# microsoft/Sora

Measured on AMD Instinct MI355X. Metric: IQ Msamples/s through 802.11a 54 Mbps RX PHY, higher is better.
Workload: dtype int16 IQ / u8 path metrics

## Files before the change

sora_amd/csrc/dev_vit16.h:

```cpp
#pragma once
#include <hip/hip_runtime.h>
#include "kernels.h"
#include "dev_viterbi.h"

namespace sora {
namespace {

template <int WIN, int LOOK> struct Geom16 {
    static constexpr int kMaxWalk = (WIN + LOOK + 7) / 8 + 2;
    static constexpr int P = kMaxWalk;
    static constexpr int kPathBytes = 40;
};

template <int WIN, int LOOK> struct Lds16 {
    uint16_t ring[Geom16<WIN, LOOK>::P][4][64];
    union {
        uint32_t udump[4][64];
        uint16_t ops[4][24][2];
        uint16_t ops2[2][4][24][2];
    };
    uint32_t path[8][Geom16<WIN, LOOK>::kPathBytes / 4];
};

constexpr unsigned kW[4] = { 0u, 21u, 42u, 63u };

__device__ __forceinline__ unsigned v_of_lane(unsigned l)
{
    const unsigned b0 = l & 1u, b1 = (l >> 1) & 1u, b2 = (l >> 2) & 1u, b3 = (l >> 3) & 1u;
    const unsigned c3 = b2, c1 = b3, c0 = b0 ^ c3, c2 = b1 ^ c3;
    return c0 | (c1 << 1) | (c2 << 2) | (c3 << 3);
}
__device__ __forceinline__ unsigned lane_of_v(unsigned v)
{
    const unsigned c0 = v & 1u, c1 = (v >> 1) & 1u, c2 = (v >> 2) & 1u, c3 = (v >> 3) & 1u;
    return c0 ^ (c2 << 1) ^ (c1 << 3) ^ (c3 ? 7u : 0u);
}
__device__ __forceinline__ unsigned rev6u(unsigned x) { return __brev(x) >> 26; }

template <int CTRL> __device__ __forceinline__ unsigned dppx(unsigned v) { return (unsigned)__builtin_amdgcn_update_dpp(0, (int)v, CTRL, 0xF, 0xF, true); }

__device__ __forceinline__ unsigned partner(unsigned v, int ph)
{
    switch (ph) {
    case 0: return dppx<0x140>(v);
    case 1: return dppx<0x1B>(v);
    case 2: return dppx<0x141>(v);
    case 3: return dppx<0x4E>(v);
    case 4: return dppx<0x128>(v);
    default: return dppx<0xB1>(v);
    }
}

struct Vit16 {
    unsigned U[4];
    unsigned MX[24];
    unsigned MY[6];
    unsigned sadr[3][4];
};

template <int WHICH, int P>
__device__ __forceinline__ void acs16(Vit16& V, int t24, unsigned a, unsigned b, unsigned pos512[3])
{
    const int ph = t24 % 6, k = t24 % 8;
    const unsigned Kp = (WHICH == 0 ? 14u : 7u) * kFld + (kOne << k);
    unsigned bm;
    if (WHICH == 0)      bm = (a ^ V.MX[t24]) + (b ^ V.MY[ph]);
    else if (WHICH == 1) bm = a ^ V.MX[t24];
    else                 bm = b ^ V.MX[t24];
    const unsigned bo = Kp - bm;
    const int rx = ph == 0 ? 2 : ph == 1 ? 1 : 0;
    unsigned N[4];
#pragma unroll
    for (int i = 0; i < 4; i++) {
        const unsigned X = V.U[i], Y = partner(V.U[i ^ rx], ph);
        const bool wb = (kW[i] >> (5 - ph)) & 1u;
        N[i] = wb ? pk_min16(X + bo, Y + bm) : pk_min16(X + bm, Y + bo);
    }
#pragma unroll
    for (int i = 0; i < 4; i++) V.U[i] = N[i];
    if (k == 7) {
        const int jb = t24 / 8;
#pragma unroll
        for (int i = 0; i < 4; i++) {
            const unsigned w = bank_word(V.U[i]);
            const unsigned addr = V.sadr[jb][i] + pos512[jb];
            asm volatile("ds_write_b16 %0, %1" : : "v"(addr), "v"(w) : "memory");
            V.U[i] &= 0xFE00FE00u;
        }
    }
}

__device__ __forceinline__ unsigned row_min_u32(unsigned v)
{
    v = min(v, dppx<0xB1>(v)); v = min(v, dppx<0x4E>(v)); v = min(v, dppx<0x141>(v)); v = min(v, dppx<0x128>(v));
    return v;
}
__device__ __forceinline__ unsigned row_pkmin(unsigned v)
{
    v = pk_min16(v, dppx<0xB1>(v)); v = pk_min16(v, dppx<0x4E>(v)); v = pk_min16(v, dppx<0x141>(v)); v = pk_min16(v, dppx<0x128>(v));
    return v;
}
__device__ __forceinline__ unsigned wave_min_u32(unsigned v) { return (unsigned)__builtin_amdgcn_readfirstlane((int)dpp_min_u32_wave(v)); }
__device__ __forceinline__ unsigned wave_max_u32(unsigned v) { return ~wave_min_u32(~v); }

template <int CR, int WIN, int LOOK, int BITS>
struct Forward16 {
    static constexpr int P = Geom16<WIN, LOOK>::P, GB = Puncture<CR>::GB, GS = Puncture<CR>::GS, CW = Puncture<CR>::CW;
    static constexpr int NV = Puncture<CR>::NV;
    struct Chunk { uint32_t v[CW]; };
    struct Raw { SoftRaw r[NV]; };

    Vit16 V;
    unsigned row, half;
    uint32_t my_j;
    SoftCursor<BITS, CW> cur[NV];
    uint32_t my_base;
    const uint8_t* soft;
    uint16_t* my_ops;
    const uint4* row_ops;
    uint32_t pos;
    unsigned pos512[3];
    uint32_t tr, nsteps;
    uint32_t next_thr;
    bool all_done;

    __device__ __forceinline__ void init(Lds16<WIN, LOOK>& S, const uint8_t* __restrict__ soft_, uint32_t my_soft_off, uint32_t my_first, uint32_t my_last, unsigned start,
                                         uint32_t nsteps_)
    {
        const unsigned lane = threadIdx.x & 63, l16 = lane & 15;
        row = lane >> 4; half = lane & 1u;
        const unsigned v0 = v_of_lane(l16);
        nsteps = nsteps_;
#pragma unroll
        for (int i = 0; i < 4; i++) V.U[i] = (v0 ^ kW[i]) == 0 ? 0u : start;
        const unsigned ring_base = (unsigned)(uintptr_t)&S.ring[0][0][0];
#pragma unroll
        for (int jb = 0; jb < 3; jb++)
#pragma unroll
            for (int i = 0; i < 4; i++) V.sadr[jb][i] = ring_base + ((row * 64u + rev6u(rol6(v0 ^ kW[i], jb == 0 ? 2 : jb == 1 ? 4 : 0))) << 1);
#pragma unroll
        for (int t = 0; t < 24; t++) {
            const int ph = t % 6, k = t % 8;
            const unsigned n = rol6(v0, ph + 1);
            const bool vb = (v0 >> (5 - ph)) & 1u;
            const unsigned ma = (__popc(n & 0155) & 1) ? 7u * kFld : 0u, mb = (__popc(n & 0117) & 1) ? 7u * kFld : 0u;
            const unsigned mx = Puncture<CR>::which_of(ph) == 2 ? mb : ma;
            V.MX[t] = vb ? ((mx ^ (7u * kFld)) | (kOne << k)) : mx;
            if (t < 6) V.MY[t] = vb ? (mb ^ (7u * kFld)) : mb;
        }
        tr = 0; pos = 0;
        my_j = l16 >> 1;
#pragma unroll
        for (int v = 0; v < NV; v++) cur[v].init(my_soft_off, my_first + my_j + 8u * v, my_last);
        my_base = my_soft_off + my_first + my_j;
        soft = soft_;
        my_ops = &S.ops[row][my_j][half];
        row_ops = reinterpret_cast<const uint4*>(&S.ops[row][0][0]);
        set_row_pos();
        clear_ops(S);
    }
    __device__ __forceinline__ bool going() const { return tr < nsteps && !all_done; }

    __device__ __forceinline__ void normalize()
    {
        const unsigned m = row_pkmin(pk_min16(pk_min16(V.U[0], V.U[1]), pk_min16(V.U[2], V.U[3])));
#pragma unroll
        for (int i = 0; i < 4; i++) V.U[i] -= m;
    }
    static __device__ __forceinline__ uint32_t pos_of(uint32_t p, int jb) { const uint32_t q = p + 512u * (uint32_t)jb; return min(q, q - 512u * (uint32_t)P); }
    __device__ __forceinline__ void set_row_pos()
    {
        pos512[0] = pos; pos512[1] = pos_of(pos, 1); pos512[2] = pos_of(pos512[1], 1);
    }
    __device__ __forceinline__ void end_row() { pos = pos_of(pos512[2], 1); set_row_pos(); }
    __device__ __forceinline__ Raw fetch(uint32_t c) const
    {
        Raw R;
#pragma unroll
        for (int v = 0; v < NV; v++) R.r[v] = cur[v].fetch(soft, c);
        return R;
    }
    __device__ __forceinline__ void put(const Raw& R, uint16_t* mine) const
    {
#pragma unroll
        for (int v = 0; v < NV; v++) soft_put(mine + 16 * v, cur[v], R.r[v]);
    }
    __device__ __forceinline__ void clear_ops(Lds16<WIN, LOOK>& S) const
    {
        if constexpr (BITS == kSoftScaled) {
            static_assert(sizeof(S.ops2) == 3 * 64 * 4, "three dwords per lane");
            uint32_t* z = reinterpret_cast<uint32_t*>(&S.ops2[0][0][0][0]) + (threadIdx.x & 63);
            z[0] = 0u; z[64] = 0u; z[128] = 0u;
            lds_fence();
        }
    }
    __device__ __forceinline__ uint32_t fast_base(uint32_t c0) const { return my_base + c0 * (uint32_t)CW; }
    template <int DC> __device__ __forceinline__ Raw fetch_at(uint32_t p) const
    {
        static_assert(BITS == kSoftScaled, "one byte per value");
        Raw R;
#pragma unroll
        for (int v = 0; v < NV; v++) { R.r[v].sh = 0; R.r[v].w = soft[(size_t)p + (size_t)(DC * CW + 8 * v)]; }
        return R;
    }
    static __device__ __forceinline__ Chunk get(const uint4* table)
    {
        Chunk K;
#pragma unroll
        for (int i = 0; i < (CW + 3) / 4; i++) {
            const uint4 x = table[i];
            K.v[4 * i] = x.x; K.v[4 * i + 1] = x.y;
            if (4 * i + 2 < CW) { K.v[4 * i + 2] = x.z; K.v[4 * i + 3] = x.w; }
        }
        return K;
    }
    __device__ __forceinline__ Chunk unpack(const Raw& R) const
    {
        put(R, my_ops);
        lds_fence();
        const Chunk K = get(row_ops);
        lds_fence();
        return K;
    }
    __device__ __forceinline__ void group(const Chunk& K, int h, int i0)
    {
        const int k0 = i0 / GS * GB, t24 = 12 * h + i0;
        acs16<0, P>(V, t24, K.v[k0], K.v[k0 + 1], pos512);
        if (CR != 0) acs16<1, P>(V, t24 + 1, K.v[k0 + 2], 0, pos512);
        if (CR == 2) acs16<2, P>(V, t24 + 2, 0, K.v[k0 + 3], pos512);
        if ((t24 + GS) % 8 == 0) normalize();
    }
    __device__ __forceinline__ void fast_chunk(const Chunk& K, int h)
    {
#pragma unroll
        for (int g = 0; g < 12 / GS; g++) group(K, h, g * GS);
        tr += 12;
    }
    template <typename CHECK> __device__ __forceinline__ void slow_chunk(const Chunk& K, int h, CHECK& check)
    {
#pragma unroll
        for (int g = 0; g < 12 / GS; g++) {
            if (going()) {
                group(K, h, g * GS);
                tr += GS;
                check(12 * h + g * GS + GS - 1);
            }
        }
    }
    template <typename CHECK> __device__ __forceinline__ void chunk(const Chunk& K, int h, CHECK& check)
    {
        if (tr + 12 <= nsteps && next_thr > tr + 12) fast_chunk(K, h); else slow_chunk(K, h, check);
    }
};

template <int WIN, int LOOK, bool LANE_OB = false>
__device__ __noinline__ void trace16(unsigned lds_off, unsigned U0, unsigned U1, unsigned U2, unsigned U3, uint32_t tr_, uint32_t ob_, uint32_t pj_, uint32_t k_,
                                     uint32_t my_cnt, uint8_t* my_out)
{
    using G = Geom16<WIN, LOOK>;
    constexpr int P = G::P, K = G::kMaxWalk;
    constexpr int NR = K - 1, NF = NR / 4, NW = K / 4 + 1;
    static_assert(NR % 4 == 0 || NR % 4 == 2, "the walk's words are packed in pairs");
    static_assert(NW * 4 <= G::kPathBytes && NW >= WIN / 32 + 1, "the stream's registers hold a window and fit Lds16::path");
    typedef __attribute__((address_space(3))) Lds16<WIN, LOOK> lds_t;
    typedef __attribute__((address_space(3))) const uint16_t lds_u16;
    lds_t& S = *(lds_t*)(uintptr_t)lds_off;
    auto uni = [](uint32_t v) { return (uint32_t)__builtin_amdgcn_readfirstlane((int)v); };
    const uint32_t tr = uni(tr_), ob = LANE_OB ? ob_ : uni(ob_), pj = uni(pj_), k = uni(k_);
    const unsigned lane = threadIdx.x & 63, row = lane >> 4, l16 = lane & 15, half = lane & 1u;
    const unsigned v0 = v_of_lane(l16);
    const unsigned U[4] = { U0, U1, U2, U3 };
    const uint32_t j = (tr - 1) >> 3, nn = tr - 8u * j, m_lo = ob >> 3;
    const unsigned rowbase = (unsigned)(uintptr_t)&S.ring[0][row][0], sh = 8u * half;
    auto ring_j = [&](unsigned idx) -> unsigned { return *(lds_u16*)(uintptr_t)(rowbase + pj + (idx << 1)); };
#pragma unroll
    for (int i = 0; i < 4; i++) S.udump[i][lane] = U[i];
    lds_fence();
    unsigned key[2] = { 0xFFFFFFFFu, 0xFFFFFFFFu };
#pragma unroll
    for (int i = 0; i < 4; i++) {
        const unsigned st = rol6(v0 ^ kW[i], tr);
        unsigned lastA, lastB;
        if (k == 7) { const unsigned w = ring_j(rev6u(st)); lastA = (w >> 7) & 1u; lastB = (w >> 15) & 1u; }
        else { lastA = (U[i] >> k) & 1u; lastB = (U[i] >> (17 + k)) & 1u; }
        const unsigned mA = ((U[i] & 0xFFFFu) >> 9 << 1) | lastA, mB = (U[i] >> 25 << 1) | lastB;
        key[0] = min(key[0], (mA << 8) | (st << 2)); key[1] = min(key[1], (mB << 8) | (st << 2));
    }
    const unsigned kA = row_min_u32(key[0]), kB = row_min_u32(key[1]);
    const unsigned st = ((half ? kB : kA) >> 2) & 0x3Fu;
    const unsigned s0 = rol6(st, 6u - tr % 6u);
    const unsigned b4 = (s0 >> 4) & 1u, b5 = (s0 >> 5) & 1u;
    const unsigned ri = b4 | (b5 << 1);
    const unsigned sl = lane_of_v((s0 ^ (b4 ? 21u : 0u) ^ (b5 ? 42u : 0u)) & 15u);
    const unsigned Ust = S.udump[ri][row * 16u + sl];
    unsigned H;
    if (nn == 8) H = (ring_j(rev6u(st)) >> sh) & 0xFFu;
    else H = ((Ust >> (17u * half)) & 0xFFu) & ((1u << nn) - 1u);
    unsigned q = rev6u(((st >> nn) | rev6u(H & 0x3Fu)) & 0x3Fu);
    unsigned pr[NR / 2];
    uint32_t p = pj;
#pragma unroll
    for (int i = 1; i < K; i++) {
        uint32_t d;
        p = __builtin_sub_overflow(p, 512u, &d) ? 512u * (uint32_t)(P - 1) : d;
        unsigned base = rowbase + p;
        asm volatile("" : "+v"(base));
        const unsigned raw = *(lds_u16*)(uintptr_t)(base + (q << 1));
        q = __builtin_amdgcn_ubfe(raw, sh, 6u);
        const int s = K - 1 - i;
        if (s & 1) pr[s >> 1] = raw << 16; else pr[s >> 1] |= raw;
    }
    unsigned R[NW];
    const unsigned sel = 0x06040200u + 0x01010101u * half;
#pragma unroll
    for (int w = 0; w < NF; w++) R[w] = __builtin_amdgcn_perm(pr[2 * w + 1], pr[2 * w], sel);
    if (NR % 4 == 0) R[NF] = H;
    else R[NF] = __builtin_amdgcn_perm(H, pr[2 * NF], 0x0C040200u + 0x00000101u * half);
    const uint32_t sfirst = (uint32_t)(K - 1) - (j - m_lo);
    bool fast = !LANE_OB;
    if (!LANE_OB) {
        const bool whole = my_cnt == (uint32_t)WIN && sfirst == 1u && (((uintptr_t)my_out + m_lo) & 3u) == 0;
        fast = __ballot(!(whole || my_cnt == 0)) == 0;
    }
    if (fast) {
        if (my_cnt != 0 && l16 < 2) {
            uint32_t* o = reinterpret_cast<uint32_t*>(my_out + m_lo);
#pragma unroll
            for (int dw = 0; dw < WIN / 32; dw++) o[dw] = __builtin_amdgcn_alignbit(R[dw + 1], R[dw], 14);
        }
    } else {
        __attribute__((address_space(3))) uint32_t* pw = S.path[row * 2u + half];
        if (l16 < 2) {
#pragma unroll
            for (int w = 0; w < NW; w++) pw[w] = R[w];
        }
        lds_fence();
        __attribute__((address_space(3))) const uint8_t* pth = (__attribute__((address_space(3))) const uint8_t*)pw;
        const uint32_t nbytes = my_cnt >> 3;
        for (uint32_t z = l16 >> 1; z < nbytes; z += 8) {
            const uint32_t sb = sfirst + z;
            my_out[m_lo + z] = (uint8_t)(((unsigned)pth[sb] >> 6) | (((unsigned)pth[sb + 1] & 0x3Fu) << 2));
        }
    }
    lds_fence();
}

}
}
```

Baseline: 55590.

## Parallelize Viterbi traceback across lanes with warm-up and speculative fix-up rounds

Result: no change. 56490 (median of 3 runs) (+1.6%).

```diff
diff --git a/sora_amd/csrc/dev_vit16.h b/sora_amd/csrc/dev_vit16.h
--- a/sora_amd/csrc/dev_vit16.h
+++ b/sora_amd/csrc/dev_vit16.h
@@ -10,6 +10,7 @@
     static constexpr int kMaxWalk = (WIN + LOOK + 7) / 8 + 2;
     static constexpr int P = kMaxWalk;
     static constexpr int kPathBytes = 40;
+    static constexpr int kWarm = 6;
 };
 
 template <int WIN, int LOOK> struct Lds16 {
@@ -297,6 +298,61 @@
     if (nn == 8) H = (ring_j(rev6u(st)) >> sh) & 0xFFu;
     else H = ((Ust >> (17u * half)) & 0xFFu) & ((1u << nn) - 1u);
     unsigned q = rev6u(((st >> nn) | rev6u(H & 0x3Fu)) & 0x3Fu);
+    const uint32_t sfirst = (uint32_t)(K - 1) - (j - m_lo);
+    if constexpr (!LANE_OB) {
+        const bool whole = my_cnt == (uint32_t)WIN && sfirst == 1u && (((uintptr_t)my_out + m_lo) & 3u) == 0;
+        if (__ballot(!(whole || my_cnt == 0)) == 0) {
+            constexpr int W = G::kWarm, ND = WIN / 32, DMAX = ND < 7 ? ND : 7, AMIN = K - 6 - 4 * DMAX, TCHK = W + 1 - AMIN;
+            static_assert(AMIN >= 1 && AMIN - W <= 1, "every dword's blocks lie at walk positions >= 1 and the topmost lane starts from the traced index");
+            const unsigned d = min(l16 >> 1, (unsigned)DMAX);
+            const int i0 = K - 6 - W - 4 * (int)d;
+            const bool true_start = i0 <= 1;
+            uint32_t p = pj + 512u * (uint32_t)(P - i0);
+            p = min(p, p - 512u * (uint32_t)P); p = min(p, p - 512u * (uint32_t)P);
+            auto step_down = [](uint32_t x) { uint32_t y; return __builtin_sub_overflow(x, 512u, &y) ? 512u * (uint32_t)(P - 1) : y; };
+            auto block = [&](uint32_t pos, unsigned idx) -> unsigned {
+                unsigned base = rowbase + pos;
+                asm volatile("" : "+v"(base));
+                return *(lds_u16*)(uintptr_t)(base + (idx << 1));
+            };
+            unsigned qs = true_start ? q : 0u, q_first = qs, q_last = 0, raw[5];
+            uint32_t p_first = p;
+#pragma unroll
+            for (int t = 0; t < W + 5; t++) {
+                if (t == W) { q_first = qs; p_first = p; }
+                if (t == W + 4) q_last = qs;
+                const unsigned r = block(p, qs), nq = __builtin_amdgcn_ubfe(r, sh, 6u);
+                qs = t < TCHK ? (i0 + t >= 1 ? nq : qs) : nq;
+                if (t >= W) raw[t - W] = r;
+                p = step_down(p);
+            }
+            const bool need = my_cnt != 0 && !true_start;
+#pragma nounroll
+            for (int round = 0; round < 7; round++) {
+                const unsigned nb = dppx<0x102>(q_last);
+                const bool bad = need && q_first != nb;
+                if (__ballot(bad) == 0) break;
+                if (bad) {
+                    q_first = nb;
+                    unsigned qq = nb;
+                    uint32_t pp = p_first;
+#pragma unroll
+                    for (int t = 0; t < 5; t++) {
+                        if (t == 4) q_last = qq;
+                        raw[t] = block(pp, qq);
+                        qq = __builtin_amdgcn_ubfe(raw[t], sh, 6u);
+                        pp = step_down(pp);
+                    }
+                }
+            }
+            if (my_cnt != 0 && (l16 >> 1) < (unsigned)ND) {
+                const unsigned lo = __builtin_amdgcn_perm((raw[1] << 16) | raw[2], (raw[3] << 16) | raw[4], half ? 0x07050301u : 0x06040200u);
+                *reinterpret_cast<uint32_t*>(my_out + m_lo + 4u * d) = __builtin_amdgcn_alignbit(__builtin_amdgcn_ubfe(raw[0], sh, 6u), lo, 6);
+            }
+            lds_fence();
+            return;
+        }
+    }
     unsigned pr[NR / 2];
     uint32_t p = pj;
 #pragma unroll
@@ -316,34 +372,20 @@
     for (int w = 0; w < NF; w++) R[w] = __builtin_amdgcn_perm(pr[2 * w + 1], pr[2 * w], sel);
     if (NR % 4 == 0) R[NF] = H;
     else R[NF] = __builtin_amdgcn_perm(H, pr[2 * NF], 0x0C040200u + 0x00000101u * half);
-    const uint32_t sfirst = (uint32_t)(K - 1) - (j - m_lo);
-    bool fast = !LANE_OB;
-    if (!LANE_OB) {
-        const bool whole = my_cnt == (uint32_t)WIN && sfirst == 1u && (((uintptr_t)my_out + m_lo) & 3u) == 0;
-        fast = __ballot(!(whole || my_cnt == 0)) == 0;
-    }
-    if (fast) {
-        if (my_cnt != 0 && l16 < 2) {
-            uint32_t* o = reinterpret_cast<uint32_t*>(my_out + m_lo);
-#pragma unroll
-            for (int dw = 0; dw < WIN / 32; dw++) o[dw] = __builtin_amdgcn_alignbit(R[dw + 1], R[dw], 14);
-        }
-    } else {
-        __attribute__((address_space(3))) uint32_t* pw = S.path[row * 2u + half];
-        if (l16 < 2) {
-#pragma unroll
-            for (int w = 0; w < NW; w++) pw[w] = R[w];
-        }
-        lds_fence();
-        __attribute__((address_space(3))) const uint8_t* pth = (__attribute__((address_space(3))) const uint8_t*)pw;
-        const uint32_t nbytes = my_cnt >> 3;
-        for (uint32_t z = l16 >> 1; z < nbytes; z += 8) {
-            const uint32_t sb = sfirst + z;
-            my_out[m_lo + z] = (uint8_t)(((unsigned)pth[sb] >> 6) | (((unsigned)pth[sb + 1] & 0x3Fu) << 2));
-        }
+    __attribute__((address_space(3))) uint32_t* pw = S.path[row * 2u + half];
+    if (l16 < 2) {
+#pragma unroll
+        for (int w = 0; w < NW; w++) pw[w] = R[w];
     }
     lds_fence();
-}
-
-}
-}
+    __attribute__((address_space(3))) const uint8_t* pth = (__attribute__((address_space(3))) const uint8_t*)pw;
+    const uint32_t nbytes = my_cnt >> 3;
+    for (uint32_t z = l16 >> 1; z < nbytes; z += 8) {
+        const uint32_t sb = sfirst + z;
+        my_out[m_lo + z] = (uint8_t)(((unsigned)pth[sb] >> 6) | (((unsigned)pth[sb + 1] & 0x3Fu) << 2));
+    }
+    lds_fence();
+}
+
+}
+}
```
